# stevenmiller888/mlx-audio

Hardware: AMD Instinct MI355X
Metric: audio-sec/sec (xRT), Kokoro-82M batch=32 fixed 128-phoneme utterances per GPU (higher is better)
Workload: dtype bf16; 1 GPU; Kokoro-82M bf16, batch=32/GPU fixed 128-phoneme utterances (T=130, F=650, 390000 samples = 16.25 s each), utterance-sharded over 1 GPU(s); global_batch=32, parallelism=utterance-shard x1, 2 batches in flight per GPU

## Files before the change

include/kokoro_hip.h:

```cpp
#ifndef KOKORO_HIP_H
#define KOKORO_HIP_H

#include <stddef.h>
#include <stdint.h>

#ifdef __cplusplus
extern "C" {
#endif

#define KK_ABI_VERSION 2
#define KK_ABI_MINOR 22

enum { KK_DTYPE_F32 = 0, KK_DTYPE_BF16 = 1, KK_DTYPE_I32 = 2, KK_DTYPE_F16 = 3 };
enum { KK_NOISE_ZERO = 0, KK_NOISE_INJECTED = 1, KK_NOISE_PHILOX = 2 };

typedef struct kk_model kk_model;
typedef struct kk_context kk_context;

typedef struct kk_config {
  int32_t n_token, hidden_dim, style_dim, n_layer, max_dur, text_encoder_kernel_size;
  int32_t plbert_hidden, plbert_heads, plbert_intermediate, plbert_max_pos, plbert_layers, plbert_embedding;
  int32_t decoder_hidden;
  int32_t upsample_initial_channel;
  int32_t n_upsamples;
  int32_t upsample_rates[4];
  int32_t upsample_kernel_sizes[4];
  int32_t n_resblock_kernels;
  int32_t resblock_kernel_sizes[4];
  int32_t resblock_dilations[4][3];
  int32_t gen_istft_n_fft, gen_istft_hop_size;
  int32_t compute_dtype;
} kk_config;

int kk_create(const kk_config* cfg, kk_model** out);
// ... 59 lines not shown
int kk_op_lstm_bf16(void* stream, int B, const float* xproj, const void* wh_bf16, int L_rows, const int32_t* len, void* out, int ldo,
                    int dtype);
int kk_op_attention(void* stream, int B, const void* qkv, int ld, int T_rows, const int32_t* len, int heads, void* out, int ldo, int dtype);
int kk_op_source_stft(void* stream, int B, const float* f0, int L2_rows, const int32_t* len2, const float* lin_w9, float lin_b,
                      int noise_mode, const float* noise, uint64_t seed, float* phase_scratch, float* har_source, void* har, int ldhar,
                      int dtype);
int kk_op_istft_head(void* stream, int B, const void* x, int ldx, int Tf_rows, const int32_t* len_frames, float* wav, int dtype, int fast);
int kk_op_pack_head_w(void* stream, const void* w_bf16, void* w_frag);
int kk_op_conv_post_istft(void* stream, int B, const void* x, int ldx, int Tf_rows, const int32_t* len_frames, const void* w_frag,
                          const float* bias, float in_slope, float* wav, void* cp_out, int cp_ld);

int kk_mxfp8_bytes(int rows, int K, size_t* q_bytes, size_t* s_bytes);
int kk_mxfp8_pack_weight(const float* w_host, int N, int K, int group, uint8_t* q_host, uint8_t* s_host);
int kk_op_linear_mxfp8(void* stream, const void* x_bf16, int ldx, int M, int rows_per_item, const int32_t* len, int K, const void* wq,
                       const void* ws, int N, const float* bias, int act, void* aq, void* as, void* out_bf16, int ldo);

int kk_debug_info(kk_context* cx, const char* name, int64_t* rows, int64_t* channels);
int kk_debug_fetch(kk_context* cx, void* stream, const char* name, float* dst);
int kk_debug_override(kk_context* cx, const char* name, const float* src);
void kk_debug_clear(kk_context* cx);
int kk_op_pack_w_frag(void* stream, const void* w_bf16, void* w_frag, int Kw, int CoutP, int CinP);
void kk_debug_set_op_wfrag(const void* w_frag);
void kk_debug_set_op_accumulate(int on);
int kk_debug_last_conv_epi(void);
void kk_debug_set_op_variant(int v);
void kk_debug_set_op_post_slope(float slope);
void kk_debug_force_generic(kk_context* cx, int flags);

int kk_profile_begin(kk_context* cx, int max_launches);
int kk_profile_end(kk_context* cx, int ncls, double* ms, double* flops, double* bytes, int64_t* count);

typedef struct kk_mimi kk_mimi;

typedef struct kk_mimi_config {
  int32_t dim, nq, bins, qdim, num_heads, num_layers, dim_feedforward, nfilters;
  int32_t n_ratios, ratios[8];
  int32_t ksize, residual_ksize, last_ksize, upsample_stride, compress;
  float rope_base;
  int32_t compute_dtype;
} kk_mimi_config;

int kk_mimi_create(const kk_mimi_config* cfg, kk_mimi** out);
void kk_mimi_destroy(kk_mimi* m);
int kk_mimi_load_tensor(kk_mimi* m, const char* name, const int64_t* shape, int ndim, const float* data);
int kk_mimi_finalize(kk_mimi* m, void* stream);
int64_t kk_mimi_samples_per_frame(const kk_mimi* m);
// ... 290 lines not shown
```

mlx-audio_amd/_lib.py:

```python
from __future__ import annotations

import ctypes as C
import os

_HERE = os.path.dirname(os.path.abspath(__file__))
LIB_PATH = os.path.join(_HERE, "libkokoro_hip.so")

KK_F32, KK_BF16, KK_I32, KK_F16 = 0, 1, 2, 3
CSM_WEIGHTS = {0: "f32", 1: "bf16", 2: "q8", 3: "q4"}
CSM_WEIGHTS_MIXED, CSM_WEIGHTS_DEQUANTIZED = 0x100, 0x200
NOISE_ZERO, NOISE_INJECTED, NOISE_PHILOX = 0, 1, 2
ACT_NONE, ACT_LRELU, ACT_GELU, ACT_SNAKE = 0, 1, 2, 3
KK_PCM_F32, KK_PCM_S16LE, KK_PCM_MULAW, KK_PCM_ALAW = 0, 1, 2, 3


class KKConfig(C.Structure):
    _fields_ = [
        ("n_token", C.c_int32), ("hidden_dim", C.c_int32), ("style_dim", C.c_int32), ("n_layer", C.c_int32),
        ("max_dur", C.c_int32), ("text_encoder_kernel_size", C.c_int32),
        ("plbert_hidden", C.c_int32), ("plbert_heads", C.c_int32), ("plbert_intermediate", C.c_int32),
        ("plbert_max_pos", C.c_int32), ("plbert_layers", C.c_int32), ("plbert_embedding", C.c_int32),
        ("decoder_hidden", C.c_int32), ("upsample_initial_channel", C.c_int32), ("n_upsamples", C.c_int32),
        ("upsample_rates", C.c_int32 * 4), ("upsample_kernel_sizes", C.c_int32 * 4),
        ("n_resblock_kernels", C.c_int32), ("resblock_kernel_sizes", C.c_int32 * 4),
# ... 240 lines not shown
    "kk_whisper_text_rows_state_bytes": (_sz, [_vp, _i]),
    "kk_whisper_text_rows_workspace_bytes": (_sz, [_vp, _i, _i]),
    "kk_whisper_text_rows_open": (_i, [_vp, _vp, _i, _vp, _sz]),
    "kk_whisper_text_rows_admit": (_i, [_vp, _vp, _i, _vp, _vp, _i, C.POINTER(KKWhisperPickParams), _vp, _vp, _sz]),
    "kk_whisper_text_rows_forward": (_i, [_vp, _vp, _vp, _i, _vp, _i, _vp, _vp, _sz]),
    "kk_whisper_text_rows_pick": (_i, [_vp, _vp, _vp, _i]),
    "kk_whisper_text_rows_flags": (_i, [_vp, _vp, _vp]),
    "kk_whisper_text_rows_read": (_i, [_vp, _vp, _i, _vp, _i, _vp, _vp]),
    "kk_whisper_text_rows_set_token": (_i, [_vp, _vp, _i, _i, _vp]),
    "kk_op_whisper_qk_rows_workspace_bytes": (_sz, [_i, _i, _i, _i]),
    "kk_op_whisper_qk_rows": (_i, [_vp, _i, _i, _i, _vp, _vp, _i, _i, _vp, _i, _i, _vp, C.c_longlong]),
    "kk_op_whisper_align_matrix_workspace_bytes": (_sz, [_i, _i, _i, _i, _i]),
    "kk_op_whisper_align_matrix": (_i, [_vp, _i, _i, _vp, C.c_longlong, C.c_longlong, _i, _vp, _i, _vp, _i, _f, _i, _i, _vp, _i, _vp, _sz]),
    "kk_op_whisper_median_filter": (_i, [_vp, C.c_longlong, _i, _vp, C.c_longlong, _i, _vp, C.c_longlong]),
    "kk_op_whisper_dtw_workspace_bytes": (_sz, [_i, _i, _i]),
    "kk_op_whisper_dtw": (_i, [_vp, _i, _vp, C.c_longlong, _i, _vp, _i, _vp, _i, _i, _vp, _vp, _vp, _vp, _vp, _sz]),
    "kk_whisper_text_qk_bytes": (_sz, [_vp, _i, _i, _i, _i]),
    "kk_whisper_text_forward_qk": (_i, [_vp, _vp, _i, _i, _vp, _vp, _vp, _i, _i, _vp, _sz, _vp, _sz]),
    "kk_mimi_debug_info": (_i, [_vp, C.c_char_p, C.POINTER(C.c_int64), C.POINTER(C.c_int64)]),
    "kk_mimi_debug_fetch": (_i, [_vp, _vp, C.c_char_p, _vp]),
    "kk_debug_set_op_wfrag": (None, [_vp]),
    "kk_debug_set_op_variant": (None, [_i]),
    "kk_debug_last_conv_epi": (_i, []),
    "kk_debug_set_op_accumulate": (None, [_i]),
    "kk_debug_set_op_post_slope": (None, [_f]),
    "kk_set_graph_mode": (_i, [_vp, _i]),
    "kk_set_quantization": (_i, [_vp, _i, _i]),
    "kk_quantized_layers": (_i, [_vp]),
    "kk_mxfp8_bytes": (_i, [_i, _i, C.POINTER(_sz), C.POINTER(_sz)]),
    "kk_mxfp8_pack_weight": (_i, [_vp, _i, _i, _i, _vp, _vp]),
    "kk_op_linear_mxfp8": (_i, [_vp, _vp, _i, _i, _i, _vp, _i, _vp, _vp, _i, _vp, _i, _vp, _vp, _vp, _i]),
    "kk_profile_begin": (_i, [_vp, _i]),
    "kk_profile_end": (_i, [_vp, _i, C.POINTER(C.c_double), C.POINTER(C.c_double), C.POINTER(C.c_double), C.POINTER(C.c_int64)]),
}

_lib = None


class KokoroHipError(RuntimeError):
    pass


def load():
    global _lib
    if _lib is not None:
        return _lib
# ... 26 lines not shown
```

mlx-audio_amd/build.py:

```python
from __future__ import annotations

import hashlib
import os
import subprocess
import sys
from concurrent.futures import ThreadPoolExecutor

HERE = os.path.dirname(os.path.abspath(__file__))
CSRC = os.path.join(HERE, "csrc")
OUT = os.path.join(HERE, "libkokoro_hip.so")
OBJ = os.path.join(HERE, "csrc", "_obj")
HIPCC = os.environ.get("HIPCC", "/opt/rocm/bin/hipcc")
FLAGS = ["-O3", "--offload-arch=gfx950", "-fPIC", "-ffp-contract=off", "-std=c++17", "-Wall", "-Wno-unused-function"]


FILE_FLAGS = {"kk_source.hip": ["-fno-slp-vectorize"], "kk_head.hip": ["-fno-slp-vectorize"], "kk_conv_mfma5.hip": ["-fno-slp-vectorize"], "kk_conv_mfma4.hip": ["-fno-slp-vectorize"], "kk_conv_mfma.hip": ["-fno-slp-vectorize"]}


def _sources():
    return sorted(f for f in os.listdir(CSRC) if f.endswith(".hip"))


def _digest() -> str:
    h = hashlib.sha256()
    for f in sorted(os.listdir(CSRC)):
        p = os.path.join(CSRC, f)
        if os.path.isfile(p) and f.endswith((".hip", ".h")):
            h.update(f.encode())
            h.update(open(p, "rb").read())
    h.update(open(os.path.join(HERE, "..", "include", "kokoro_hip.h"), "rb").read())
    h.update(" ".join(FLAGS).encode())
    h.update(repr(sorted(FILE_FLAGS.items())).encode())
    return h.hexdigest()


def build(force: bool = False, verbose: bool = True, extra_flags=(), out: str = OUT, obj_dir: str = OBJ) -> str:
    OUT, OBJ = out, obj_dir
    stamp = os.path.join(OBJ, "digest.txt")
    dig = _digest() + " ".join(extra_flags)
# ... 32 lines not shown
```

mlx-audio_amd/csrc/kk_kernels.h:

```cpp
#pragma once
#include "kk_common.h"

int kk_launch_conv_generic(const KKConvArgs& a, int B, int in_dtype, int out_dtype, hipStream_t st);

struct KKMfmaArgs {
  const bf16_t* x;
  long long xbs;
  int ldx;
  const bf16_t* w;
  const bf16_t* wf;
  int CinP, CoutP;
  int Cin;
  const float* bias;
  void* out;
  long long obs;
  int ldo;
  const void* res;
  long long rbs;
  int ldr;
  int Cout;
  int Kw, mode, stride, pad, dil, in_shift;
  int Q, Lo_rows;
  KKLen lin, lout;
  float in_slope, scale;
// ... 32 lines not shown
};
__host__ __device__ inline long long kk_linear_pack_index(int o, int i, int K) {
  return (((long long)(o >> 4) * (K >> 5) + (i >> 5)) * 64 + ((i & 31) >> 3) * 16 + (o & 15)) * 8 + (i & 7);
}
int kk_launch_linear_rows_mfma(const KKLinMfmaArgs& a, hipStream_t st);
bool kk_mfma_eligible(int Cin, int Cout, int Kw, int mode, int stride, int dil);
constexpr int KK_MFMA_TILE_ROWS = 192;
int kk_launch_conv_mfma(const KKMfmaArgs& a, int B, int out_dtype, hipStream_t st);
int kk_launch_conv_mfma4(const KKMfmaArgs& a, int B, int out_dtype, hipStream_t st);
bool kk_mfma4_wholek_eligible(const KKMfmaArgs& a);
bool kk_mfma5_eligible(const KKMfmaArgs& a, int out_dtype);
int kk_launch_conv_mfma5(const KKMfmaArgs& a, int B, int out_dtype, hipStream_t st);
extern int kk_conv_epi_generic, kk_conv_epi_last;
#define KK_MFMA4_PACK_INDEX(tap, cout, k, CoutP, CinP)                                                              \
  ({                                                                                                                \
    const int nbk = (cout) / 128, cr = (cout) % 128, chunk = (k) / 64, kr = (k) % 64;                               \
    const long long blk = ((long long)(tap) * ((CoutP) / 128) + nbk) * ((CinP) / 64) + chunk;                       \
    const int wc = cr / 64, ni = (cr % 64) / 16, ks = kr / 32, kq = (kr % 32) / 8, j = kr % 8;                      \
    const int lane = kq * 16 + (cr % 16);                                                                           \
    blk * (128 * 64) + ((long long)(((wc * 2 + ks) * 4 + ni) * 64 + lane)) * 8 + j;                                 \
  })
inline long long kk_mfma4_pack_index(int tap, int cout, int k, int CoutP, int CinP) { return KK_MFMA4_PACK_INDEX(tap, cout, k, CoutP, CinP); }
int kk_launch_pack_w_frag(const void* w, void* wf, int Kw, int CoutP, int CinP, hipStream_t st);

struct KKStatsArgs {
  const float* gb;
  int gbs;
  float* pa;
  float* pb;
  int pstride, Cp;
  int fused;
  const void* x;
  long long xbs;
  int ldx;
  int C;
  int Lmax;
  KKLen len;
  float* partial;
  int nchunk;
  int rows_per_chunk;
  float* mean;
  float* rstd;
  float eps;
};
size_t kk_stats_partial_floats(int B, int C, int Lmax, int rows_per_chunk);
int kk_launch_instnorm_stats(KKStatsArgs a, int B, int dtype, hipStream_t st);
// ... 194 lines not shown
```

mlx-audio_amd/csrc/kk_model.hip:

```cpp
#include <math.h>
#include <stdio.h>
#include <string.h>

#include <algorithm>
#include <functional>
#include <map>
#include <string>
#include <vector>

#include "../../include/kokoro_hip.h"
#include "kk_common.h"
#include "kk_kernels.h"
#include "kk_host.h"

static thread_local std::string g_err;
static const void* g_op_wfrag = nullptr;
static float g_op_post_slope = 0.f;
static int g_op_variant = 4;
static int g_op_accumulate = 0;
int kk_conv_epi_generic = 0;
int kk_conv_epi_last = -1;

int kk_fail(const char* msg) {
  g_err = msg ? msg : "unknown error";
  return -1;
}
extern "C" const char* kk_last_error(void) { return g_err.c_str(); }
extern "C" int kk_abi_version(void) { return KK_ABI_VERSION; }
extern "C" int kk_abi_minor(void) { return KK_ABI_MINOR; }

namespace {

struct ConvW {
  size_t w_off = 0, b_off = 0;
  bool has_bias = false;
  int Cin = 0, Cout = 0, Kw = 0, ldw = 0;
  const float* w = nullptr;
  const float* b = nullptr;
  bool mfma = false;
  size_t wb_off = 0, wf_off = 0;
  int CinP = 0, CoutP = 0, Cout8 = 0;
  const bf16_t* wb = nullptr;
  const bf16_t* wf = nullptr;
  size_t wl_off = 0;
// ... 71 lines not shown
  kk_model* m = nullptr;
  DebugNotes dbg;
  std::map<std::string, const float*> dbg_over;

  int flags = 0;
  bool force_generic = false;
  bool no_fusion = false;
  bool prof_on = false;
  std::vector<hipEvent_t> prof_ev;
  bool graph_mode = false;
  GraphCache graphs{16};
  unsigned long long* seed_dev = nullptr;
  bool capturing = false;
  bool no_v4 = false;
  bool no_fp8 = false;
  int v5_mode = 0;
  bool no_head_fusion = false;
  bool keep_debug = false;
  hipStream_t side_stream = nullptr;
  hipEvent_t side_fork[2] = {nullptr, nullptr}, side_join[2] = {nullptr, nullptr};
  bool no_side = false;
  bool no_wholek = false;
  int linrows_mode = 0;
  struct ProfRec { int cls; double flops; double bytes; };
  std::vector<ProfRec> prof_rec;
};

extern "C" int kk_create(const kk_config* cfg, kk_model** out) {
  if (!cfg || !out) return kk_fail("kk_create: null argument");
  if (cfg->n_upsamples != 2 || cfg->n_resblock_kernels < 1 || cfg->n_resblock_kernels > 4)
    return kk_fail("kk_create: unsupported generator geometry");
  if (cfg->plbert_hidden != cfg->plbert_heads * 64) return kk_fail("kk_create: Albert head size must be 64");
  if (cfg->style_dim != 128) return kk_fail("kk_create: style_dim must be 128 (kokoro.py:145,165 split ref_s at 128)");
  if (cfg->hidden_dim % 32 != 0 || cfg->hidden_dim / 2 > 256) return kk_fail("kk_create: hidden_dim must be a multiple of 32, <= 512");
  if (cfg->gen_istft_n_fft != 20 || cfg->gen_istft_hop_size != 5) return kk_fail("kk_create: iSTFT head is built for n_fft 20 / hop 5");
  if (cfg->compute_dtype != KK_DTYPE_F32 && cfg->compute_dtype != KK_DTYPE_BF16) return kk_fail("kk_create: compute_dtype");
  kk_model* m = new (std::nothrow) kk_model();
  if (!m) return kk_fail("kk_create: out of memory");
  m->cfg = *cfg;
  m->adt = cfg->compute_dtype == KK_DTYPE_BF16 ? KK_BF16 : KK_F32;
  *out = m;
  return 0;
}

extern "C" void kk_destroy(kk_model* m) {
  if (!m) return;
// ... 637 lines not shown
    if (o.res) { a.res = o.res->p; a.rbs = o.res->bs; a.ldr = o.res->ld; }
    a.Cin = w.Cin; a.Cout = w.Cout; a.Kw = w.Kw;
    a.mode = o.mode; a.stride = o.stride; a.pad = o.pad; a.dil = o.dil; a.in_shift = o.in_shift;
    a.Q = Q; a.Lo_rows = out.rows;
    a.lin = lin; a.lout = lout;
    a.in_slope = o.in_slope; a.scale = o.scale; a.accumulate = o.accumulate; a.act = o.act; a.act_slope = o.act_slope;
    const double rows_out = o.mode == KK_CONVT ? (double)Q * o.stride : (double)Q;
    const double taps = o.mode == KK_CONVT ? (double)w.Kw / o.stride : (double)w.Kw;
    const double flops = 2.0 * B * rows_out * w.Cout * (o.alg_taps_cin > 0 ? o.alg_taps_cin : w.Cin * taps);
    const double bytes = B * (rows_out * w.Cout * esz(out.dtype) * (o.res ? 2.0 : 1.0) + (double)Q * (o.mode == KK_CONVT ? 1 : o.stride) * w.Cin * esz(x.dtype)) +
                         (double)w.Kw * w.Cin * w.Cout * 4.0;
    if (can_fp8(w, x, lin, out, lout, Q, o)) {
      KKFp8Args f;
      memset(&f, 0, sizeof f);
      f.aq = (const uint4*)q8_aq; f.as = (const unsigned char*)q8_as; f.wq = w.q8; f.ws = w.s8;
      f.M = B * x.rows; f.N = w.Cout; f.K = w.Cin; f.bias = w.b; f.out = (bf16_t*)out.p; f.ldo = out.ld; f.rows_per_item = x.rows;
      f.lout = lout; f.act = o.act;
      prof_start();
      int rc = kk_launch_mxfp8_quant_rows(x.p, x.ld, f.M, f.K, q8_aq, q8_as, st);
      if (rc == 0) rc = kk_launch_linear_mxfp8(f, st);
      prof_stop(10, flops, B * (double)Q * (w.Cin * 2.0 + w.Cin * 1.03 * 2.0 + w.Cout * 2.0) + (double)w.Cin * w.Cout * 1.03);
      return rc;
    }
    const bool lr_size_ok = cx->linrows_mode == 1 || (cx->linrows_mode == 0 && (long long)B * Q <= 1024);
    if (lr_size_ok && w.wl && w.Kw == 1 && can_mfma(w, x, out, o) && out.dtype == KK_BF16 && o.mode == KK_CONV && o.stride == 1 && o.pad == 0 && o.dil == 1 &&
        o.in_shift == 0 && !o.nrm_a && !o.want_stats && !o.res && !o.accumulate && o.in_slope == 1.f && o.scale == 1.f && o.post_slope == 1.f &&
        (o.act == KK_ACT_NONE || o.act == KK_ACT_GELU) && Q == x.rows && Q == out.rows && lin.len == lout.len && lin.mul == lout.mul && lin.add == lout.add &&
        !cx->no_v4) {
      KKLinMfmaArgs f;
      memset(&f, 0, sizeof f);
      f.x = (const bf16_t*)x.p; f.xbs = x.bs; f.ldx = x.ld; f.wl = w.wl; f.bias = w.b; f.Nb = w.CoutP;
      f.out = (bf16_t*)out.p; f.obs = out.bs; f.ldo = out.ld; f.K = w.Cin; f.N = w.Cout8; f.rows = Q; f.items = B;
      f.flat = (x.bs == (long long)x.rows * x.ld && out.bs == (long long)out.rows * out.ld) ? 1 : 0;
      f.len = lout; f.act = o.act;
      prof_start();
      const int rc = kk_launch_linear_rows_mfma(f, st);
      prof_stop(1, flops, bytes);
      return rc;
    }
    if (can_mfma(w, x, out, o)) {
      KKMfmaArgs g;
      memset(&g, 0, sizeof g);
      g.nrm_a = o.nrm_a; g.nrm_b = o.nrm_b; g.nrm_stride = fz_stride; g.nrm_act = o.nrm_act; g.nrm_slope = o.nrm_slope;
      g.nrm_alpha = o.nrm_alpha; g.nrm_C = o.nrm_C;
      g.x = (const bf16_t*)x.p; g.xbs = x.bs; g.ldx = x.ld; g.w = w.wb; g.CinP = w.CinP; g.Cin = w.Cin; g.CoutP = w.CoutP; g.bias = w.b;
      g.out = out.p; g.obs = out.bs; g.ldo = out.ld;
      if (o.res) { g.res = o.res->p; g.rbs = o.res->bs; g.ldr = o.res->ld; }
// ... 2 lines not shown
      g.act = o.act; g.act_slope = o.act_slope; g.post_slope = o.post_slope;
      if (o.want_stats) {
        last_ntiles = kk_cdiv(Q, KK_MFMA_TILE_ROWS) * (o.mode == KK_CONVT ? o.stride : 1);
        if ((size_t)B * last_ntiles * 2 * w.Cout > fz_part_floats) return kk_fail("internal: statistics scratch too small");
        g.stat_part = fz_part;
        g.stat_ntiles = last_ntiles;
      }
      const bool v4 = w.wf && out.dtype == KK_BF16 && !cx->no_v4;
      g.wf = v4 ? w.wf : nullptr;
      const bool v5 = v4 && cx->v5_mode != 2 && (cx->v5_mode == 1 || g.Kw >= 9 || (g.Kw >= 7 && g.CinP >= 256)) && B <= 256 && kk_mfma5_eligible(g, out.dtype);
      g.slabwise = (cx->no_wholek || (!g.nrm_a && g.CinP < 192)) ? 1 : 0;
      int Bl = B;
      if (!v5 && B > 1 && w.Kw == 1 && o.mode == KK_CONV && o.stride == 1 && o.pad == 0 && o.dil == 1 && o.in_shift == 0 && !o.nrm_a && !o.want_stats &&
          Q == x.rows && Q == out.rows && Q % 192 != 0 && x.bs == (long long)x.rows * x.ld && out.bs == (long long)out.rows * out.ld &&
          (!o.res || (o.res->rows == out.rows && o.res->bs == (long long)o.res->rows * o.res->ld)) && (long long)B * Q < (1ll << 30)) {
        g.flat_T = Q;
        g.flat_len = lout;
        g.Q = B * Q;
        g.Lo_rows = B * out.rows;
        g.lin = KKLen{nullptr, 0, B * Q};
        g.lout = KKLen{nullptr, 0, B * Q};
        Bl = 1;
      }
      prof_start();
      const int rc = v5 ? kk_launch_conv_mfma5(g, Bl, out.dtype, st) : v4 ? kk_launch_conv_mfma4(g, Bl, out.dtype, st) : kk_launch_conv_mfma(g, Bl, out.dtype, st);
      prof_stop(1, flops, bytes);
      return rc;
    }
    if (o.nrm_a || o.want_stats) return kk_fail("internal: fused norm requested on a conv that is not MFMA eligible");
    prof_start();
    const int rc = kk_launch_conv_generic(a, B, x.dtype, out.dtype, st);
    prof_stop(0, flops, bytes);
    return rc;
  }

  void* q8_aq = nullptr;
  void* q8_as = nullptr;
  size_t q8_rows = 0, q8_K = 0;
  bool can_fp8(const ConvW& w, const Buf& x, KKLen lin, const Buf& out, KKLen lout, int Q, const ConvOpt& o) const {
    return w.fp8 && !cx->no_fp8 && !cx->force_generic && q8_aq && x.dtype == KK_BF16 && out.dtype == KK_BF16 && w.Kw == 1 && o.mode == KK_CONV &&
           o.stride == 1 && o.pad == 0 && o.dil == 1 && o.in_shift == 0 && o.in_slope == 1.f && !o.res && o.scale == 1.f && !o.accumulate &&
           (o.act == KK_ACT_NONE || o.act == KK_ACT_GELU) && !o.nrm_a && !o.want_stats && x.rows == out.rows && Q == x.rows &&
           x.bs == (long long)x.rows * x.ld && out.bs == (long long)out.rows * out.ld && x.ld % 8 == 0 && !((uintptr_t)x.p & 15) &&
           lin.len == lout.len && lin.mul == lout.mul && lin.add == lout.add && (size_t)B * x.rows <= q8_rows && (size_t)w.Cin <= q8_K;
  }

  bool can_mfma(const ConvW& w, const Buf& x, const Buf& out, const ConvOpt& o) const {
    const bool al16 = !(((uintptr_t)x.p | (uintptr_t)out.p | (uintptr_t)(o.res ? o.res->p : nullptr)) & 15);
// ... 622 lines not shown
extern "C" int kk_forward(kk_context* cx, void* stream, int B, int Tmax, const int32_t* ids, const int32_t* lens, const float* ref_s,
                          const float* speed, const int32_t* forced_dur, int Fmax, int noise_mode, const float* sine_noise, uint64_t seed,
                          void* workspace, size_t workspace_bytes, float* wav_out, int32_t* pred_dur_out, int32_t* nframes_out) {
  if (!cx) return kk_fail("kk_forward: null context");
  kk_model* m = cx->m;
  KK_TRY(check_common(m, B, Tmax, "kk_forward"));
  if (!ids || !lens || !ref_s || !speed || !wav_out || Fmax <= 0) return kk_fail("kk_forward: bad argument");
  if (noise_mode == KK_NOISE_INJECTED && !sine_noise) return kk_fail("kk_forward: KK_NOISE_INJECTED needs sine_noise");
  if (workspace_bytes < kk_context_workspace_bytes(cx, B, Tmax, Fmax)) return kk_fail("kk_forward: workspace too small");
  auto eager = [&](void* on_stream) -> int {
    Ctx c;
    KK_TRY(make_ctx(cx, on_stream, B, workspace, workspace_bytes, c));
    TextState ts;
    KK_TRY(run_text(c, Tmax, ids, lens, ref_s, speed, ts, pred_dur_out));
    return run_audio(c, Tmax, lens, ref_s, forced_dur ? forced_dur : ts.pred_dur, Fmax, noise_mode, sine_noise, seed, ts, wav_out, nframes_out);
  };
  if (!cx->graph_mode || cx->prof_on || !cx->dbg_over.empty()) return eager(stream);
  hipStream_t st = (hipStream_t)stream;
  const std::vector<unsigned long long> key = {(unsigned long long)B, (unsigned long long)Tmax, (unsigned long long)Fmax,
      (unsigned long long)noise_mode, (unsigned long long)(uintptr_t)ids, (unsigned long long)(uintptr_t)lens,
      (unsigned long long)(uintptr_t)ref_s, (unsigned long long)(uintptr_t)speed, (unsigned long long)(uintptr_t)forced_dur,
      (unsigned long long)(uintptr_t)sine_noise, (unsigned long long)(uintptr_t)workspace, (unsigned long long)workspace_bytes,
      (unsigned long long)(uintptr_t)wav_out, (unsigned long long)(uintptr_t)pred_dur_out, (unsigned long long)(uintptr_t)nframes_out,
      (unsigned long long)(unsigned)cx->flags};
  if (!cx->seed_dev && hipMalloc((void**)&cx->seed_dev, 8) != hipSuccess) return kk_fail("kk_forward: hipMalloc(seed) failed");
  auto work = [&](hipStream_t on_stream, bool capturing) -> int {
    cx->capturing = capturing;
    const int rc = eager((void*)on_stream);
    cx->capturing = false;
    return rc;
  };
  hipGraphExec_t ex = nullptr;
  KK_TRY(cx->graphs.run(key, st, work, &ex, "kk_forward"));
  if (!ex) return 0;
  KK_TRY(kk_launch_set_u64(cx->seed_dev, seed, st));
  if (hipGraphLaunch(ex, st) != hipSuccess) return kk_fail("kk_forward: hipGraphLaunch failed");
  return 0;
}

extern "C" int kk_set_graph_mode(kk_context* cx, int on) {
  if (!cx) return kk_fail("kk_set_graph_mode: null context");
  cx->graph_mode = on != 0;
  return 0;
}

extern "C" int kk_op_conv1d(void* stream, int B, const void* x, int ldx, int Lin_rows, const int32_t* lin, const float* w_packed, int ldw,
                            const float* bias, int Cin, int Cout, int Kw, int transposed, int stride, int pad, int dil, int in_shift,
// ... 133 lines not shown
namespace {
__global__ void pack_linear_kernel(const bf16_t* w, bf16_t* wl, int N, int K) {
  const long long n = (long long)((N + 15) / 16 * 16) * K;
  for (long long e = (long long)blockIdx.x * 256 + threadIdx.x; e < n; e += (long long)gridDim.x * 256) {
    const int o = (int)(e / K), i = (int)(e - (long long)o * K);
    wl[kk_linear_pack_index(o, i, K)] = o < N ? w[(long long)o * K + i] : (bf16_t)0.f;
  }
}
}
extern "C" int kk_op_linear_rows(void* stream, int B, const void* x_bf16, long long xbs, int ldx, int rows, const int32_t* len, const void* w_bf16, int N, int K,
                                 const float* bias, int act, void* pack_scratch, void* out_bf16, long long obs, int ldo) {
  if (!x_bf16 || !w_bf16 || !pack_scratch || !out_bf16 || B < 1 || rows < 1 || K % 32 || N % 2) return kk_fail("kk_op_linear_rows: bad argument");
  hipLaunchKernelGGL(pack_linear_kernel, dim3(256), dim3(256), 0, (hipStream_t)stream, (const bf16_t*)w_bf16, (bf16_t*)pack_scratch, N, K);
  KK_CHECK_LAUNCH();
  KKLinMfmaArgs f;
  memset(&f, 0, sizeof f);
  f.x = (const bf16_t*)x_bf16; f.xbs = xbs; f.ldx = ldx; f.wl = (const bf16_t*)pack_scratch; f.bias = bias; f.Nb = N;
  f.out = (bf16_t*)out_bf16; f.obs = obs; f.ldo = ldo; f.K = K; f.N = N; f.rows = rows; f.items = B;
  f.flat = (xbs == (long long)rows * ldx && obs == (long long)rows * ldo) ? 1 : 0;
  f.len = KKLen{len, len ? 1 : 0, len ? 0 : rows}; f.act = act;
  return kk_launch_linear_rows_mfma(f, (hipStream_t)stream);
}

extern "C" int kk_op_attention(void* stream, int B, const void* qkv, int ld, int T_rows, const int32_t* len, int heads, void* out, int ldo,
                               int dtype) {
  KKAttnArgs a;
  memset(&a, 0, sizeof a);
  a.qkv = qkv; a.bs = (long long)T_rows * ld; a.ld = ld; a.out = out; a.obs = (long long)T_rows * ldo; a.ldo = ldo; a.heads = heads;
  a.hs = heads * 64; a.Tmax = T_rows; a.len = KKLen{len, len ? 1 : 0, len ? 0 : T_rows}; a.scale = 0.125f;
  return kk_launch_attention(a, B, dtype, (hipStream_t)stream);
}

extern "C" int kk_op_source_stft(void* stream, int B, const float* f0, int L2_rows, const int32_t* len2, const float* lin_w9, float lin_b,
                                 int noise_mode, const float* noise, uint64_t seed, float* phase_scratch, float* har_source, void* har,
                                 int ldhar, int dtype) {
  KKSourceArgs sa;
  memset(&sa, 0, sizeof sa);
  sa.f0 = f0; sa.L2max = L2_rows; sa.len2 = len2; sa.phase = phase_scratch; sa.lin_w = lin_w9; sa.lin_b = lin_b; sa.noise = noise;
  sa.seed = seed; sa.noise_mode = noise_mode; sa.har_source = har_source; sa.Nmax = 300 * L2_rows; sa.upsample = 300;
  KK_TRY(kk_launch_source(sa, B, (hipStream_t)stream));
  if (len2) return kk_fail("kk_op_source_stft: ragged lengths are exercised through kk_forward only");
  const int Tf = 60 * L2_rows + 1;
  return kk_launch_stft20(har_source, sa.Nmax, nullptr, har, (long long)Tf * ldhar, ldhar, Tf, B, dtype, (hipStream_t)stream);
}

extern "C" int kk_op_istft_head(void* stream, int B, const void* x, int ldx, int Tf_rows, const int32_t* len_frames, float* wav, int dtype,
// ... 73 lines not shown
  if (!w_host || !q_host || !s_host) return kk_fail("kk_mxfp8_pack_weight: null argument");
  return kk_mxfp8_pack_weight_host(w_host, N, K, group, q_host, s_host);
}
extern "C" int kk_op_linear_mxfp8(void* stream, const void* x_bf16, int ldx, int M, int rows_per_item, const int32_t* len, int K,
                                  const void* wq, const void* ws, int N, const float* bias, int act, void* aq, void* as, void* out_bf16,
                                  int ldo) {
  if (!x_bf16 || !wq || !ws || !aq || !as || !out_bf16) return kk_fail("kk_op_linear_mxfp8: null argument");
  KK_TRY(kk_launch_mxfp8_quant_rows(x_bf16, ldx, M, K, aq, as, (hipStream_t)stream));
  KKFp8Args f;
  memset(&f, 0, sizeof f);
  f.aq = (const uint4*)aq; f.as = (const unsigned char*)as; f.wq = (const uint4*)wq; f.ws = (const unsigned char*)ws;
  f.M = M; f.N = N; f.K = K; f.bias = bias; f.out = (bf16_t*)out_bf16; f.ldo = ldo; f.rows_per_item = rows_per_item;
  f.lout = KKLen{len, len ? 1 : 0, len ? 0 : rows_per_item};
  f.act = act;
  return kk_launch_linear_mxfp8(f, (hipStream_t)stream);
}
extern "C" void kk_debug_set_op_wfrag(const void* w_frag) { g_op_wfrag = w_frag; }
extern "C" void kk_debug_set_op_post_slope(float slope) { g_op_post_slope = slope; }
extern "C" void kk_debug_set_op_variant(int v) {
  kk_conv_epi_generic = (v == 41 || v == 51) ? 1 : 0;
  g_op_variant = (v == 5 || v == 51) ? 5 : v == 40 ? 40 : 4;
}
extern "C" int kk_debug_last_conv_epi(void) { return kk_conv_epi_last; }
extern "C" void kk_debug_set_op_accumulate(int on) { g_op_accumulate = on ? 1 : 0; }
extern "C" int kk_op_pack_w_frag(void* stream, const void* w_bf16, void* w_frag, int Kw, int CoutP, int CinP) {
  return kk_launch_pack_w_frag(w_bf16, w_frag, Kw, CoutP, CinP, (hipStream_t)stream);
}
extern "C" void kk_debug_clear(kk_context* cx) {
  if (!cx) return;
  cx->dbg_over.clear();
  cx->dbg.map.clear();
}

extern "C" int kk_profile_begin(kk_context* cx, int max_launches) {
  if (!cx || max_launches <= 0) return kk_fail("kk_profile_begin: bad argument");
  while ((int)cx->prof_ev.size() < 2 * max_launches) {
    hipEvent_t e;
    if (hipEventCreate(&e) != hipSuccess) return kk_fail("kk_profile_begin: hipEventCreate failed");
    cx->prof_ev.push_back(e);
  }
  cx->prof_rec.clear();
  cx->prof_on = true;
  return 0;
}
extern "C" int kk_profile_end(kk_context* cx, int ncls, double* ms, double* flops, double* bytes, int64_t* count) {
  if (!cx || !ms || !flops || !bytes || !count) return kk_fail("kk_profile_end: null argument");
// ... 13 lines not shown
```

Before: 15750 audio-sec/sec.

## Add LDS-direct global-load linear kernel with triple-buffered ring for 1x1 bf16 linears

Adds a new MFMA linear kernel for pointwise (Kw=1) bf16 projections. It streams activation and fragment-ordered weight slabs straight into LDS via global_load_lds in a three-deep ring, uses XCD-aware block remapping, and interleaves MFMAs with the loads through scheduling barriers. By default it is routed only for large row counts (B*Q > 1024) and only when the grid fits within one wave of CUs, replacing the mfma4 conv path for those calls. The goal is to hide global-memory latency and cut register staging for the larger linears. The cost is extra code, a 1-block-per-CU launch bound, and routing heuristics that may miss shapes.

New measurement: 15390 audio-sec/sec. 0.977x the previous value.

```diff
diff --git a/include/kokoro_hip.h b/include/kokoro_hip.h
--- a/include/kokoro_hip.h
+++ b/include/kokoro_hip.h
@@ -9,7 +9,7 @@
 #endif
 
 #define KK_ABI_VERSION 2
-#define KK_ABI_MINOR 22
+#define KK_ABI_MINOR 23
 
 enum { KK_DTYPE_F32 = 0, KK_DTYPE_BF16 = 1, KK_DTYPE_I32 = 2, KK_DTYPE_F16 = 3 };
 enum { KK_NOISE_ZERO = 0, KK_NOISE_INJECTED = 1, KK_NOISE_PHILOX = 2 };
@@ -115,6 +115,10 @@
 int kk_op_pack_w_frag(void* stream, const void* w_bf16, void* w_frag, int Kw, int CoutP, int CinP);
 void kk_debug_set_op_wfrag(const void* w_frag);
 void kk_debug_set_op_accumulate(int on);
+void kk_debug_set_linear_glds(kk_context* cx, int mode);
+int kk_debug_last_linear_glds(void);
+int kk_op_linear_tiled_bf16(void* stream, int B, const void* x_bf16, int ldx, int rows, const int32_t* len, int CinP, int CoutP, const float* bias, int Cout,
+                            int act, void* out_bf16, int ldo, int flat);
 int kk_debug_last_conv_epi(void);
 void kk_debug_set_op_variant(int v);
 void kk_debug_set_op_post_slope(float slope);
diff --git a/mlx-audio_amd/_lib.py b/mlx-audio_amd/_lib.py
--- a/mlx-audio_amd/_lib.py
+++ b/mlx-audio_amd/_lib.py
@@ -286,6 +286,9 @@
     "kk_debug_set_op_wfrag": (None, [_vp]),
     "kk_debug_set_op_variant": (None, [_i]),
     "kk_debug_last_conv_epi": (_i, []),
+    "kk_debug_set_linear_glds": (None, [_vp, _i]),
+    "kk_debug_last_linear_glds": (_i, []),
+    "kk_op_linear_tiled_bf16": (_i, [_vp, _i, _vp, _i, _i, _vp, _i, _i, _vp, _i, _i, _vp, _i, _i]),
     "kk_debug_set_op_accumulate": (None, [_i]),
     "kk_debug_set_op_post_slope": (None, [_f]),
     "kk_set_graph_mode": (_i, [_vp, _i]),
diff --git a/mlx-audio_amd/build.py b/mlx-audio_amd/build.py
--- a/mlx-audio_amd/build.py
+++ b/mlx-audio_amd/build.py
@@ -14,7 +14,7 @@
 FLAGS = ["-O3", "--offload-arch=gfx950", "-fPIC", "-ffp-contract=off", "-std=c++17", "-Wall", "-Wno-unused-function"]
 
 
-FILE_FLAGS = {"kk_source.hip": ["-fno-slp-vectorize"], "kk_head.hip": ["-fno-slp-vectorize"], "kk_conv_mfma5.hip": ["-fno-slp-vectorize"], "kk_conv_mfma4.hip": ["-fno-slp-vectorize"], "kk_conv_mfma.hip": ["-fno-slp-vectorize"]}
+FILE_FLAGS = {"kk_source.hip": ["-fno-slp-vectorize"], "kk_head.hip": ["-fno-slp-vectorize"], "kk_conv_mfma5.hip": ["-fno-slp-vectorize"], "kk_conv_mfma4.hip": ["-fno-slp-vectorize"], "kk_conv_mfma.hip": ["-fno-slp-vectorize"], "kk_linear_glds.hip": ["-fno-slp-vectorize"]}
 
 
 def _sources():
diff --git a/mlx-audio_amd/csrc/kk_kernels.h b/mlx-audio_amd/csrc/kk_kernels.h
--- a/mlx-audio_amd/csrc/kk_kernels.h
+++ b/mlx-audio_amd/csrc/kk_kernels.h
@@ -78,6 +78,10 @@
   })
 inline long long kk_mfma4_pack_index(int tap, int cout, int k, int CoutP, int CinP) { return KK_MFMA4_PACK_INDEX(tap, cout, k, CoutP, CinP); }
 int kk_launch_pack_w_frag(const void* w, void* wf, int Kw, int CoutP, int CinP, hipStream_t st);
+bool kk_linear_glds_eligible(const KKMfmaArgs& a, int out_dtype);
+int kk_launch_linear_glds(const KKMfmaArgs& a, int B, hipStream_t st);
+bool kk_linear_glds_routed(const KKMfmaArgs& a, int B);
+extern int kk_linear_glds_last;
 
 struct KKStatsArgs {
   const float* gb;
diff --git a/mlx-audio_amd/csrc/kk_linear_glds.hip b/mlx-audio_amd/csrc/kk_linear_glds.hip
--- /dev/null
+++ b/mlx-audio_amd/csrc/kk_linear_glds.hip
@@ -0,0 +1,253 @@
+#include "kk_common.h"
+#include "kk_kernels.h"
+#include "kk_conv_mfma_shared.h"
+
+int kk_linear_glds_last = 0;
+
+namespace {
+
+constexpr int LG_BN = 128, LG_CK = 64, LG_CLD = 132;
+constexpr int LG_WSLAB = LG_BN * LG_CK * 2;
+constexpr int LG_MI = 4, LG_NBUF = 3;
+
+template <int MI, int NBUF>
+struct LgGeo {
+  static constexpr int WM = MI * 16, BM = 2 * WM;
+  static constexpr int XSLAB = BM * 128, SLAB = XSLAB + LG_WSLAB, RING = NBUF * SLAB, CS = BM * LG_CLD * 4;
+  static constexpr int LDS_BYTES = RING > CS ? RING : CS;
+  static constexpr int NX = BM / 32, NL = NX + 4;
+};
+
+#define LG_VMCNT(N) asm volatile("s_waitcnt vmcnt(%0)" ::"n"(N) : "memory")
+#define LG_BAR()                                       \
+  {                                                    \
+    asm volatile("s_waitcnt lgkmcnt(0)" ::: "memory"); \
+    __builtin_amdgcn_s_barrier();                      \
+  }
+#define LG_GPTR(p) ((const __attribute__((address_space(1))) void*)(p))
+#define LG_LPTR(p) ((__attribute__((address_space(3))) void*)(p))
+
+template <int MI, int NBUF, int ACT>
+__global__ __launch_bounds__(256, 1) void linear_glds_kernel(KKMfmaArgs a) {
+  using G = LgGeo<MI, NBUF>;
+  constexpr int WM = G::WM, BM = G::BM, NX = G::NX, NL = G::NL, PF = NBUF - 1;
+  static_assert(NBUF >= 2 && NBUF <= 4, "ring depth");
+  extern __shared__ __attribute__((aligned(16))) unsigned char smem[];
+
+  const int tid = threadIdx.x, lane = tid & 63, wave = __builtin_amdgcn_readfirstlane(tid >> 6);
+  const int wr = wave >> 1, wc = wave & 1;
+  int bx, by, b;
+  {
+    const int gx = gridDim.x, gy = gridDim.y, total = gx * gy * gridDim.z;
+    int lid = blockIdx.x + gx * (blockIdx.y + gy * blockIdx.z);
+    const int per = total / 8, rem = total - per * 8;
+    const int xcd = lid & 7, idx = lid >> 3;
+    lid = xcd * per + (xcd < rem ? xcd : rem) + idx;
+    by = lid % gy;
+    const int t = lid / gy;
+    bx = t % gx;
+    b = t / gx;
+  }
+  const int q0 = bx * BM, n0 = by * LG_BN;
+  const int Lout = kk_len(a.lout, b);
+  const bool tile_live = q0 < Lout;
+
+  kk_f32x4 acc[MI][4];
+#pragma unroll
+  for (int i = 0; i < MI; ++i)
+#pragma unroll
+    for (int j = 0; j < 4; ++j) acc[i][j] = kk_f32x4{0.f, 0.f, 0.f, 0.f};
+
+  if (tile_live) {
+    const int nchunk = a.CinP / LG_CK;
+    const bf16_t* xsrc[NX];
+#pragma unroll
+    for (int j = 0; j < NX; ++j) {
+      const int row = (wave * NX + j) * 8 + (lane >> 3);
+      const int q = q0 + row < a.Q ? q0 + row : a.Q - 1;
+      xsrc[j] = a.x + (long long)b * a.xbs + (long long)q * a.ldx + 8 * ((lane & 7) ^ ((row >> 1) & 7));
+    }
+    const bf16_t* wsrc = a.wf + (long long)by * nchunk * (LG_BN * LG_CK) + (wave * 4) * 512 + lane * 8;
+    auto issue1 = [&](int i, int c, int s) __attribute__((always_inline)) {
+      unsigned char* buf = smem + s * G::SLAB;
+      if (i < NX) __builtin_amdgcn_global_load_lds(LG_GPTR(xsrc[i] + c * LG_CK), LG_LPTR(buf + (wave * NX + i) * 1024), 16, 0, 0);
+      else
+        __builtin_amdgcn_global_load_lds(LG_GPTR(wsrc + (long long)c * (LG_BN * LG_CK) + (i - NX) * 512), LG_LPTR(buf + G::XSLAB + (wave * 4 + i - NX) * 1024), 16, 0,
+                                         0);
+    };
+    auto issue = [&](int c, int s) __attribute__((always_inline)) {
+#pragma unroll
+      for (int i = 0; i < NL; ++i) issue1(i, c, s);
+    };
+    const int sw = (lane & 15) >> 1;
+    const int aoff0 = (wr * WM + (lane & 15)) * 128 + (((lane >> 4)) ^ sw) * 16;
+    const int aoff1 = (wr * WM + (lane & 15)) * 128 + ((4 + (lane >> 4)) ^ sw) * 16;
+    const int boff = G::XSLAB + (wc * 2) * 4 * 1024 + lane * 16;
+
+#pragma unroll
+    for (int p = 0; p < PF; ++p) issue(p, p);
+    int s = 0, sn = PF;
+#pragma unroll 1
+    for (int c = 0; c < nchunk; ++c) {
+      LG_VMCNT((PF - 1) * NL);
+      LG_BAR();
+      const unsigned char* buf = smem + s * G::SLAB;
+      kk_bf16x8 bv[2][4], av[2][MI];
+#pragma unroll
+      for (int ks = 0; ks < 2; ++ks) {
+#pragma unroll
+        for (int ni = 0; ni < 4; ++ni) bv[ks][ni] = *(const kk_bf16x8*)(buf + boff + (ks * 4 + ni) * 1024);
+#pragma unroll
+        for (int mi = 0; mi < MI; ++mi) av[ks][mi] = *(const kk_bf16x8*)(buf + (ks ? aoff1 : aoff0) + mi * 2048);
+      }
+      __builtin_amdgcn_sched_barrier(0);
+      issue(c + PF < nchunk ? c + PF : nchunk - 1, sn);
+#pragma unroll
+      for (int ks = 0; ks < 2; ++ks)
+#pragma unroll
+        for (int mi = 0; mi < MI; ++mi)
+#pragma unroll
+          for (int ni = 0; ni < 4; ++ni) acc[mi][ni] = __builtin_amdgcn_mfma_f32_16x16x32_bf16(av[ks][mi], bv[ks][ni], acc[mi][ni], 0, 0, 0);
+#pragma unroll
+      for (int g = 0; g < 2 * MI; ++g) {
+        __builtin_amdgcn_sched_group_barrier(0x008, 4, 0);
+        if (g < NL) __builtin_amdgcn_sched_group_barrier(0x020, 1, 0);
+      }
+      __builtin_amdgcn_sched_barrier(0);
+      s = s + 1 == NBUF ? 0 : s + 1;
+      sn = sn + 1 == NBUF ? 0 : sn + 1;
+    }
+    LG_VMCNT(0);
+    LG_BAR();
+  }
+
+  float* Cs = (float*)smem;
+  bf16_t* ob = (bf16_t*)a.out + (long long)b * a.obs;
+  const int n = n0 + (tid & 15) * 8;
+  unsigned livemask = 0;
+  {
+    if (a.flat_T) {
+      int lens[BM / 16];
+#pragma unroll
+      for (int j = 0; j < BM / 16; ++j) {
+        const int q = q0 + j * 16 + (tid >> 4), qc = q < a.Lo_rows ? q : a.Lo_rows - 1;
+        lens[j] = qc / a.flat_T;
+      }
+      if (a.flat_len.len) {
+#pragma unroll
+        for (int j = 0; j < BM / 16; ++j) lens[j] = a.flat_len.len[lens[j]];
+#pragma unroll
+        for (int j = 0; j < BM / 16; ++j) lens[j] = lens[j] * a.flat_len.mul + a.flat_len.add;
+      } else {
+#pragma unroll
+        for (int j = 0; j < BM / 16; ++j) lens[j] = a.flat_len.add;
+      }
+#pragma unroll
+      for (int j = 0; j < BM / 16; ++j) {
+        const int q = q0 + j * 16 + (tid >> 4), qc = q < a.Lo_rows ? q : a.Lo_rows - 1;
+        const bool live = tile_live && q < Lout && (qc - (qc / a.flat_T) * a.flat_T) < lens[j];
+        livemask |= live ? 1u << j : 0u;
+      }
+    } else {
+#pragma unroll
+      for (int j = 0; j < BM / 16; ++j) livemask |= (tile_live && q0 + j * 16 + (tid >> 4) < Lout) ? 1u << j : 0u;
+    }
+  }
+  v2f bias2[4];
+  if (a.bias) {
+#pragma unroll
+    for (int k = 0; k < 4; ++k) bias2[k] = v2f{a.bias[n + 2 * k], a.bias[n + 2 * k + 1]};
+  } else {
+#pragma unroll
+    for (int k = 0; k < 4; ++k) bias2[k] = v2f{0.f, 0.f};
+  }
+  if (tile_live) {
+#pragma unroll
+    for (int mi = 0; mi < MI; ++mi)
+#pragma unroll
+      for (int ni = 0; ni < 4; ++ni) {
+        const int col = wc * 64 + ni * 16 + (lane & 15);
+        const int rbase = wr * WM + mi * 16 + 4 * (lane >> 4);
+#pragma unroll
+        for (int r = 0; r < 4; ++r) Cs[(rbase + r) * LG_CLD + col] = acc[mi][ni][r];
+      }
+    __syncthreads();
+  }
+#pragma unroll
+  for (int j = 0; j < BM / 16; ++j) {
+    const int row = j * 16 + (tid >> 4);
+    const int q = q0 + row;
+    v2f v[4];
+    if (tile_live) {
+      const float4 c0 = *(const float4*)(Cs + row * LG_CLD + (tid & 15) * 8);
+      const float4 c1 = *(const float4*)(Cs + row * LG_CLD + (tid & 15) * 8 + 4);
+      v[0] = v2f{c0.x, c0.y}; v[1] = v2f{c0.z, c0.w}; v[2] = v2f{c1.x, c1.y}; v[3] = v2f{c1.z, c1.w};
+    } else {
+#pragma unroll
+      for (int k = 0; k < 4; ++k) v[k] = v2f{0.f, 0.f};
+    }
+#pragma unroll
+    for (int k = 0; k < 4; ++k) v[k] += bias2[k];
+    if (ACT == KK_ACT_GELU) {
+#pragma unroll
+      for (int k = 0; k < 4; ++k) {
+        v[k].x = gelu_exact(v[k].x);
+        v[k].y = gelu_exact(v[k].y);
+      }
+    }
+    if (!((livemask >> j) & 1)) {
+#pragma unroll
+      for (int k = 0; k < 4; ++k) v[k] = v2f{0.f, 0.f};
+    }
+    unsigned w4[4];
+#pragma unroll
+    for (int k = 0; k < 4; ++k) {
+      typedef __bf16 lg_bf2 __attribute__((ext_vector_type(2)));
+      const lg_bf2 pk = {(bf16_t)v[k].x, (bf16_t)v[k].y};
+      w4[k] = __builtin_bit_cast(unsigned, pk);
+    }
+    if (q < a.Q && q < a.Lo_rows && n < a.Cout) *(uint4*)(ob + (long long)q * a.ldo + n) = make_uint4(w4[0], w4[1], w4[2], w4[3]);
+  }
+}
+
+template <int MI, int NBUF, int ACT>
+int launch_glds(const KKMfmaArgs& a, int B, hipStream_t st) {
+  using G = LgGeo<MI, NBUF>;
+  static KKDevOnce attr_once;
+  if (attr_once.first()) {
+    (void)hipFuncSetAttribute((const void*)linear_glds_kernel<MI, NBUF, ACT>, hipFuncAttributeMaxDynamicSharedMemorySize, G::LDS_BYTES);
+    attr_once.done();
+  }
+  dim3 grid(kk_cdiv(a.Q, G::BM), a.CoutP / LG_BN, B);
+  hipLaunchKernelGGL((linear_glds_kernel<MI, NBUF, ACT>), grid, dim3(256), G::LDS_BYTES, st, a);
+  KK_CHECK_LAUNCH();
+  return 0;
+}
+
+}
+
+bool kk_linear_glds_eligible(const KKMfmaArgs& a, int out_dtype) {
+  return a.wf && out_dtype == KK_BF16 && a.mode == KK_CONV && a.Kw == 1 && a.stride == 1 && a.pad == 0 && a.dil == 1 && a.in_shift == 0 && !a.nrm_a &&
+         !a.stat_part && !a.res && !a.accumulate && a.in_slope == 1.f && a.in_act == 0 && a.scale == 1.f && (a.post_slope == 0.f || a.post_slope == 1.f) &&
+         (a.act == KK_ACT_NONE || a.act == KK_ACT_GELU) && a.CinP >= 3 * LG_CK && a.CinP % LG_CK == 0 && a.CoutP % LG_BN == 0 &&
+         (a.Cin == 0 || a.Cin == a.CinP) && a.Cout % 8 == 0 && a.ldx >= a.CinP && a.ldx % 8 == 0 && a.ldo % 8 == 0 && a.xbs % 8 == 0 && a.obs % 8 == 0 &&
+         !(((uintptr_t)a.x | (uintptr_t)a.out | (uintptr_t)a.wf) & 15) && a.Q > 0 && a.Lo_rows >= a.Q;
+}
+
+bool kk_linear_glds_routed(const KKMfmaArgs& a, int B) {
+  static int cus[64];
+  int dev = 0;
+  if (hipGetDevice(&dev) != hipSuccess || dev < 0 || dev >= 64) return false;
+  if (!cus[dev]) {
+    int n = 0;
+    if (hipDeviceGetAttribute(&n, hipDeviceAttributeMultiprocessorCount, dev) != hipSuccess || n <= 0) return false;
+    cus[dev] = n;
+  }
+  return (long long)kk_cdiv(a.Q, LgGeo<LG_MI, LG_NBUF>::BM) * (a.CoutP / LG_BN) * B <= cus[dev];
+}
+
+int kk_launch_linear_glds(const KKMfmaArgs& a, int B, hipStream_t st) {
+  if (B <= 0 || !kk_linear_glds_eligible(a, KK_BF16)) return kk_fail("linear_glds: launch not eligible");
+  kk_linear_glds_last = 1;
+  return a.act == KK_ACT_GELU ? launch_glds<LG_MI, LG_NBUF, KK_ACT_GELU>(a, B, st) : launch_glds<LG_MI, LG_NBUF, KK_ACT_NONE>(a, B, st);
+}
diff --git a/mlx-audio_amd/csrc/kk_model.hip b/mlx-audio_amd/csrc/kk_model.hip
--- a/mlx-audio_amd/csrc/kk_model.hip
+++ b/mlx-audio_amd/csrc/kk_model.hip
@@ -20,6 +20,7 @@
 static int g_op_accumulate = 0;
 int kk_conv_epi_generic = 0;
 int kk_conv_epi_last = -1;
+static int g_op_glds = 0;
 
 int kk_fail(const char* msg) {
   g_err = msg ? msg : "unknown error";
@@ -137,6 +138,7 @@
   bool no_side = false;
   bool no_wholek = false;
   int linrows_mode = 0;
+  int glds_mode = 0;
   struct ProfRec { int cls; double flops; double bytes; };
   std::vector<ProfRec> prof_rec;
 };
@@ -820,7 +822,8 @@
       prof_stop(10, flops, B * (double)Q * (w.Cin * 2.0 + w.Cin * 1.03 * 2.0 + w.Cout * 2.0) + (double)w.Cin * w.Cout * 1.03);
       return rc;
     }
-    const bool lr_size_ok = cx->linrows_mode == 1 || (cx->linrows_mode == 0 && (long long)B * Q <= 1024);
+    const bool lr_size_ok = (cx->linrows_mode == 1 || (cx->linrows_mode == 0 && (long long)B * Q <= 1024)) &&
+                            !(cx->glds_mode == 1 && w.wf && w.CinP >= 192 && w.Cin == w.CinP);
     if (lr_size_ok && w.wl && w.Kw == 1 && can_mfma(w, x, out, o) && out.dtype == KK_BF16 && o.mode == KK_CONV && o.stride == 1 && o.pad == 0 && o.dil == 1 &&
         o.in_shift == 0 && !o.nrm_a && !o.want_stats && !o.res && !o.accumulate && o.in_slope == 1.f && o.scale == 1.f && o.post_slope == 1.f &&
         (o.act == KK_ACT_NONE || o.act == KK_ACT_GELU) && Q == x.rows && Q == out.rows && lin.len == lout.len && lin.mul == lout.mul && lin.add == lout.add &&
@@ -869,8 +872,14 @@
         g.lout = KKLen{nullptr, 0, B * Q};
         Bl = 1;
       }
+      bool glds = false;
+      if (v4 && !v5 && Q == x.rows && Q == out.rows && kk_linear_glds_eligible(g, out.dtype)) {
+        glds = cx->glds_mode == 1 || (cx->glds_mode == 0 && !cx->no_wholek && (long long)B * Q > 1024 && kk_linear_glds_routed(g, Bl));
+        if (!glds) kk_linear_glds_last = 2;
+      }
       prof_start();
-      const int rc = v5 ? kk_launch_conv_mfma5(g, Bl, out.dtype, st) : v4 ? kk_launch_conv_mfma4(g, Bl, out.dtype, st) : kk_launch_conv_mfma(g, Bl, out.dtype, st);
+      const int rc = glds ? kk_launch_linear_glds(g, Bl, st)
+                     : v5 ? kk_launch_conv_mfma5(g, Bl, out.dtype, st) : v4 ? kk_launch_conv_mfma4(g, Bl, out.dtype, st) : kk_launch_conv_mfma(g, Bl, out.dtype, st);
       prof_stop(1, flops, bytes);
       return rc;
     }
@@ -1539,7 +1548,8 @@
       (unsigned long long)(uintptr_t)ref_s, (unsigned long long)(uintptr_t)speed, (unsigned long long)(uintptr_t)forced_dur,
       (unsigned long long)(uintptr_t)sine_noise, (unsigned long long)(uintptr_t)workspace, (unsigned long long)workspace_bytes,
       (unsigned long long)(uintptr_t)wav_out, (unsigned long long)(uintptr_t)pred_dur_out, (unsigned long long)(uintptr_t)nframes_out,
-      (unsigned long long)(unsigned)cx->flags};
+      (unsigned long long)(unsigned)cx->flags,
+      (unsigned long long)cx->linrows_mode, (unsigned long long)cx->glds_mode};
   if (!cx->seed_dev && hipMalloc((void**)&cx->seed_dev, 8) != hipSuccess) return kk_fail("kk_forward: hipMalloc(seed) failed");
   auto work = [&](hipStream_t on_stream, bool capturing) -> int {
     cx->capturing = capturing;
@@ -1719,6 +1729,33 @@
   return kk_launch_linear_rows_mfma(f, (hipStream_t)stream);
 }
 
+extern "C" int kk_op_linear_tiled_bf16(void* stream, int B, const void* x_bf16, int ldx, int rows, const int32_t* len, int CinP, int CoutP, const float* bias,
+                                       int Cout, int act, void* out_bf16, int ldo, int flat) {
+  if (!x_bf16 || !out_bf16 || !g_op_wfrag || B < 1 || rows < 1 || CinP % 64 || CoutP % 128 || Cout % 8 || Cout > CoutP || ldx < CinP || ldo < Cout)
+    return kk_fail("kk_op_linear_tiled_bf16: bad argument (the fragment-order weights are set with kk_debug_set_op_wfrag)");
+  if (!kk_mfma_eligible(CinP, Cout, 1, KK_CONV, 1, 1)) return kk_fail("kk_op_linear_tiled_bf16: shape not eligible for the MFMA kernel");
+  KKMfmaArgs g;
+  memset(&g, 0, sizeof g);
+  g.x = (const bf16_t*)x_bf16; g.xbs = (long long)rows * ldx; g.ldx = ldx; g.wf = (const bf16_t*)g_op_wfrag; g.CinP = CinP; g.CoutP = CoutP; g.bias = bias;
+  g.out = out_bf16; g.obs = (long long)rows * ldo; g.ldo = ldo; g.Cout = Cout; g.Kw = 1; g.mode = KK_CONV; g.stride = 1; g.dil = 1;
+  g.Q = rows; g.Lo_rows = rows;
+  g.lin = KKLen{len, len ? 1 : 0, len ? 0 : rows};
+  g.lout = g.lin;
+  g.in_slope = 1.f; g.scale = 1.f; g.act = act;
+  int Bl = B;
+  if (flat) {
+    if ((long long)B * rows >= (1ll << 30)) return kk_fail("kk_op_linear_tiled_bf16: too many flat rows");
+    g.flat_T = rows; g.flat_len = g.lout; g.Q = B * rows; g.Lo_rows = B * rows;
+    g.lin = KKLen{nullptr, 0, B * rows};
+    g.lout = g.lin;
+    Bl = 1;
+  }
+  if (g_op_glds == 1) return kk_launch_linear_glds(g, Bl, (hipStream_t)stream);
+  kk_linear_glds_last = 2;
+  g.slabwise = g_op_variant == 40;
+  return kk_launch_conv_mfma4(g, Bl, KK_BF16, (hipStream_t)stream);
+}
+
 extern "C" int kk_op_attention(void* stream, int B, const void* qkv, int ld, int T_rows, const int32_t* len, int heads, void* out, int ldo,
                                int dtype) {
   KKAttnArgs a;
@@ -1838,6 +1875,16 @@
   g_op_variant = (v == 5 || v == 51) ? 5 : v == 40 ? 40 : 4;
 }
 extern "C" int kk_debug_last_conv_epi(void) { return kk_conv_epi_last; }
+extern "C" void kk_debug_set_linear_glds(kk_context* cx, int mode) {
+  const int m = (mode == 1 || mode == 2) ? mode : 0;
+  if (cx) cx->glds_mode = m;
+  else g_op_glds = m;
+}
+extern "C" int kk_debug_last_linear_glds(void) {
+  const int v = kk_linear_glds_last;
+  kk_linear_glds_last = 0;
+  return v;
+}
 extern "C" void kk_debug_set_op_accumulate(int on) { g_op_accumulate = on ? 1 : 0; }
 extern "C" int kk_op_pack_w_frag(void* stream, const void* w_bf16, void* w_frag, int Kw, int CoutP, int CinP) {
   return kk_launch_pack_w_frag(w_bf16, w_frag, Kw, CoutP, CinP, (hipStream_t)stream);
```
